# Jaroan/Contracts-MARL-AAM-Corridors

Hardware: AMD Instinct MI355X
Metric: env-steps/sec (whole node) at 4096 envs x 10 agents, navigation_graph (higher is better)
Workload: dtype f64

## Files before the change

contracts-marl-aam-corridors_amd/csrc/gmpe_kernel.h:

```cpp
#pragma once
#include <hip/hip_runtime.h>
#include <math.h>
#include <stdio.h>
#include <stdlib.h>
#include <string.h>

#include <string>
#include <utility>
#include <vector>

#include "gmpe_device.h"

namespace gmpe {

enum { MODE_STEP = 0, MODE_RESET = 1 };
enum { SC_NAV = 0, SC_NAV_WALLS = 1, SC_JULY = 2, SC_ROT = 3, SC_TWO = 4, SC_THREE = 5, SC_COUNT = 6 };
__host__ __device__ constexpr bool sc_kinematic(int sc) { return sc >= SC_JULY; }
__host__ __device__ constexpr bool sc_rotfam(int sc) { return sc >= SC_ROT; }
__host__ __device__ constexpr bool sc_phasefam(int sc) { return sc == SC_TWO || sc == SC_THREE; }

struct KParams {
    gmpe_config c;
    DevState s;
    gmpe_outputs o;
// ... 224 lines not shown
        base = k;
        const int64_t kk = k + i;
        double val;
        if (p.s.tape) val = kk < p.s.tape_len ? p.s.tape[(size_t)n * p.s.tape_len + kk] : __builtin_nan("");
        else val = philox_uniform(p.c.seed, (uint32_t)(p.c.env_id_base + n), (uint64_t)kk);
        __builtin_amdgcn_fence(__ATOMIC_ACQUIRE, "wavefront");
        buf[i] = val;
        __builtin_amdgcn_fence(__ATOMIC_RELEASE, "wavefront");
        __builtin_amdgcn_wave_barrier();
        __builtin_amdgcn_fence(__ATOMIC_ACQUIRE, "wavefront");
    }
    double v = buf[(int)(k - base)];
    if (v != v) { err |= 1; v = 0.5; }
    return v;
}

__device__ __forceinline__ bool closer_than(double dx, double dy, double thr) {
    const double d2 = dx * dx + dy * dy, t2 = thr * thr;
    if (d2 < t2 * (1.0 - 1e-12)) return true;
    if (d2 > t2 * (1.0 + 1e-12)) return false;
    return sqrt(d2) < thr;
}
__device__ __forceinline__ double draw_raw(const KParams& p, int n, int64_t k) {
    if (p.s.tape) return k < p.s.tape_len ? p.s.tape[(size_t)n * p.s.tape_len + k] : 0.5;
    return philox_uniform(p.c.seed, (uint32_t)(p.c.env_id_base + n), (uint64_t)k);
}
__device__ __forceinline__ void wave_lds_sync() {
    __builtin_amdgcn_fence(__ATOMIC_RELEASE, "wavefront");
    __builtin_amdgcn_wave_barrier();
    __builtin_amdgcn_fence(__ATOMIC_ACQUIRE, "wavefront");
}
struct DrawBuf { const double* d; int64_t base; int nd; };
__device__ __forceinline__ double buf_get(const KParams& p, const DrawBuf& w, int n, int64_t k) {
    const int64_t o = k - w.base;
    return o < w.nd ? w.d[o] : draw_raw(p, n, k);
}
__device__ __forceinline__ void place_uniform(const KParams& p, const Lds& l, const DrawBuf& win, int n, int i, bool mine, unsigned long long emask, int M, int base, double thr,
                                              bool check_static, bool is_agent, int64_t& ctr, int& err) {
    const gmpe_config& c = p.c;
    const int A = p.A, O = p.O, o0 = p.A + p.L;
    const double ws = c.world_size, size = c.entity_size, lo = -ws / 2, hi = ws / 2;
    const int lane0 = emask ? __ffsll((long long)emask) - 1 : 0;
    double* cx = l.vox; double* cy = l.voy;
    unsigned long long* cm = reinterpret_cast<unsigned long long*>(l.vnx);
    int k = 0, tries = 0;
    while (__ballot(mine && k < M)) {
        if (mine && k < M) {
            const double px = 0.8 * (lo + (hi - lo) * buf_get(p, win, n, ctr + 2 * i));
            const double py = 0.8 * (lo + (hi - lo) * buf_get(p, win, n, ctr + 2 * i + 1));
            bool bad0 = false;
            if (check_static) {
                bad0 = wall_band_hit(p, px, py, size);
                for (int o = 0; o < O; ++o) bad0 = bad0 || closer_than(l.ex[o0 + o] - px, l.ey[o0 + o] - py, 2.0 * (size + size));
            }
            for (int q = 0; q < k; ++q) bad0 = bad0 || closer_than(l.ex[base + q] - px, l.ey[base + q] - py, thr);
            cx[i] = px; cy[i] = py;
            wave_lds_sync();
            unsigned long long cl = 0ull;
            for (int j = 0; j < i; ++j) if (closer_than(cx[j] - px, cy[j] - py, thr)) cl |= 1ull << j;
            cm[i] = cl;
            wave_lds_sync();
            const unsigned long long bad = (__ballot(bad0) & emask) >> lane0;
            unsigned long long acc = 0ull;
            int kk = k, t = tries, used = 0, slot = -1;
            for (int j = 0; j < A && kk < M; ++j) {
                const bool b = ((bad >> j) & 1ull) || (cm[j] & acc) != 0ull;
                used = j + 1;
                if (b && ++t < GMPE_MAX_TRIES) continue;
                if (b) err |= 2;
                if (j == i) slot = kk;
                acc |= 1ull << j; ++kk; t = 0;
            }
            wave_lds_sync();
            if (slot >= 0) {
                l.ex[base + slot] = px; l.ey[base + slot] = py;
                if (is_agent) { l.n2[slot] = 0.0; l.n3[slot] = 0.0; }
            }
            wave_lds_sync();
            ctr += 2 * used; k = kk; tries = t;
        }
    }
}

template <int SC, bool BATCH = false>
__device__ __forceinline__ void reset_world_coop(const KParams& p, const Lds& l, int n, int i, bool mine, unsigned long long emask, int64_t& ctr, int& err) {
    const gmpe_config& c = p.c;
    const double ws = c.world_size, size = c.entity_size;
    const int A = p.A, L = p.L, O = p.O;
    const int o0 = A + L;
    int64_t wbase = -(int64_t)A - 1;
    const int64_t ctr_in = ctr;
    const DrawBuf win = {reinterpret_cast<const double*>(l.M), ctr, BATCH ? (p.E * p.E + 3) / 4 * 2 : 0};
    const int lane0 = emask ? __ffsll((long long)emask) - 1 : 0;
#define WDRAW(k) (BATCH ? buf_get(p, win, n, (k)) : win_draw(p, l.serr, wbase, A, n, i, (k), err))
    if (sc_kinematic(SC)) {
        double entx = 0, enty = 0, exx = 0, exy = 0, sa = 0, ca = 1;
        if (mine) {
            (void)WDRAW(ctr++);
            const double a = 3 * size * 2.5, b = ws * 0.15;
            const double width = a > b ? a : b;
            const double angle = -M_PI / 2 + (M_PI / 2 - (-M_PI / 2)) * WDRAW(ctr++);
            double tl = ws * 0.8;
            if (sc_phasefam(SC)) tl += -ws * 0.3 + (ws * 0.1 - (-ws * 0.3)) * WDRAW(ctr++);
            ca = cos(angle); sa = sin(angle);
            const double be = tl / 4, bx = -tl / 4;
            entx = ca * 0 + sa * be; enty = -sa * 0 + ca * be;
            exx = ca * 0 + sa * bx; exy = -sa * 0 + ca * bx;
            const double dx = exx - entx, dy = exy - enty;
            const double Lt = sqrt(dx * dx + dy * dy) + 1e-9;
            const double ex = dx / Lt, ey = dy / Lt;
            if (i == 0) {
                double* t = l.tube;
                t[T_ANGLE] = angle; t[T_ENTX] = entx; t[T_ENTY] = enty; t[T_EXX] = exx; t[T_EXY] = exy;
                t[T_EX] = ex; t[T_EY] = ey; t[T_NX] = (double)(float)(-ey); t[T_NY] = (double)(float)ex;
                t[T_L] = Lt; t[T_HALFW] = width * 0.5; t[T_WIDTH] = width;
                for (int q = 0; q < GMPE_TUBE_STRIDE; ++q) p.s.tube[(size_t)n * GMPE_TUBE_STRIDE + q] = t[q];
            }
        }
        int k = 0, tries = 0;
        double mx = 0, my = 0;
        if constexpr (BATCH) while (__ballot(mine && k < A)) {
            if (mine && k < A) {
                const double u0 = buf_get(p, win, n, ctr + 2 * i), u1 = buf_get(p, win, n, ctr + 2 * i + 1);
                constexpr bool rot = sc_rotfam(SC);
                const double jf = rot ? 0.3 : 0.2;
                const double jx = jf * (-ws + (ws - (-ws)) * u0), jy = jf * (-ws + (ws - (-ws)) * u1);
                const double dfe = rot ? (ws + k) / 3 : (ws + k) / 5;
                const double px = entx + dfe * sa + jx, py = enty + dfe * ca + jy;
                bool bad_i = wall_band_hit(p, px, py, size);
                for (int o = 0; o < O; ++o) bad_i = bad_i || closer_than(l.ex[o0 + o] - px, l.ey[o0 + o] - py, 2.0 * (size + size));
                for (int q = 0; q < k; ++q) bad_i = bad_i || closer_than(l.ex[q] - px, l.ey[q] - py, c.sep_dist);
                const unsigned long long all = emask >> lane0;
                const unsigned long long good = ~((__ballot(bad_i) & emask) >> lane0) & all;
                const int jg = good ? __ffsll((long long)good) - 1 : A;
                const int jfo = GMPE_MAX_TRIES - 1 - tries;
                int js;
                if (jfo < A && jfo < jg) { js = jfo; err |= 2; }
                else if (jg < A) js = jg;
                else { tries += A; ctr += 2 * A; continue; }
                ctr += 2 * (js + 1);
                const double th = 0.0 + (2 * M_PI - 0.0) * buf_get(p, win, n, ctr); ++ctr;
                if (i == js) { l.ex[k] = px; l.ey[k] = py; l.n2[k] = th; l.n3[k] = c.v_min; }
                wave_lds_sync();
                ++k; tries = 0;
            }
        }
        else while (__ballot(mine && k < A)) {
            if (mine && k < A) {
                const double u0 = WDRAW(ctr), u1 = WDRAW(ctr + 1);
                ctr += 2;
                constexpr bool rot = sc_rotfam(SC);
                const double jf = rot ? 0.3 : 0.2;
                const double jx = jf * (-ws + (ws - (-ws)) * u0), jy = jf * (-ws + (ws - (-ws)) * u1);
                const double dfe = rot ? (ws + k) / 3 : (ws + k) / 5;
                const double px = entx + dfe * sa + jx, py = enty + dfe * ca + jy;
                bool bad_i = wall_band_hit(p, px, py, size);
                for (int o = i; o < O; o += A) bad_i = bad_i || norm2(l.ex[o0 + o] - px, l.ey[o0 + o] - py) < 2.0 * (size + size);
                bad_i = bad_i || (i < k && norm2(mx - px, my - py) < c.sep_dist);
                const bool bad = (__ballot(bad_i) & emask) != 0ull;
                if (bad && ++tries < GMPE_MAX_TRIES) continue;
                if (bad) err |= 2;
                const double th = 0.0 + (2 * M_PI - 0.0) * WDRAW(ctr++);
                if (i == k) { mx = px; my = py; l.ex[k] = px; l.ey[k] = py; l.n2[k] = th; l.n3[k] = c.v_min; }
                ++k; tries = 0;
            }
        }
        if (mine) {
            if (c.formation_type == GMPE_FORMATION_LINE) {
                const int div = L - 1;
                const double s0 = -ws / 2, e0 = ws / 2, ddx = e0 - s0, ddy = s0 - s0;
                for (int q = i; q < L; q += A) {
                    const double f = div > 0 ? (double)q / (double)div : (double)q;
                    double lx = f * ddx + s0, ly = f * ddy + s0;
                    if (L > 1 && q == L - 1) { lx = e0; ly = s0; }
                    bool hit = wall_band_hit(p, lx, ly, size);
                    for (int o = 0; o < O; ++o) hit = hit || norm2(l.ex[o0 + o] - lx, l.ey[o0 + o] - ly) < 2.0 * (size + size);
                    if (hit) err |= 2;
                    l.ex[A + q] = lx; l.ey[A + q] = ly;
                }
            } else if (c.formation_type == GMPE_FORMATION_CIRCLE) {
                const double cy = exy + ws / 5, radius = ws / 3, angle_step = 2 * M_PI / L;
                for (int q = i; q < L; q += A) {
                    const double ang = q * angle_step;
                    l.ex[A + q] = 0.0 + radius * cos(ang); l.ey[A + q] = cy + radius * sin(ang);
                }
            } else {
                const double rel = -ws / 3;
                const double rx = ca * 0.0 + sa * rel, ry = -sa * 0.0 + ca * rel;
                for (int q = i; q < L; q += A) { l.ex[A + q] = exx + rx; l.ey[A + q] = exy + ry; }
            }
        }
    } else if constexpr (BATCH) {
        place_uniform(p, l, win, n, i, mine, emask, O, o0, 2.0 * (size + size), false, false, ctr, err);
        place_uniform(p, l, win, n, i, mine, emask, A, 0, c.sep_dist, true, true, ctr, err);
        place_uniform(p, l, win, n, i, mine, emask, L, A, c.sep_dist, true, false, ctr, err);
        if (mine) for (int o = i; o < O; o += A) {
            p.s.obstacles[((size_t)n * O + o) * 2] = l.ex[o0 + o];
            p.s.obstacles[((size_t)n * O + o) * 2 + 1] = l.ey[o0 + o];
        }
    } else {
        const double lo = -ws / 2, hi = ws / 2;
        int k = 0, tries = 0;
        while (__ballot(mine && k < O)) {
            if (mine && k < O) {
                const double px = 0.8 * (lo + (hi - lo) * WDRAW(ctr));
                const double py = 0.8 * (lo + (hi - lo) * WDRAW(ctr + 1));
                ctr += 2;
                bool bad_i = false;
                for (int q = i; q < k; q += A) bad_i = bad_i || norm2(l.ex[o0 + q] - px, l.ey[o0 + q] - py) < 2.0 * (size + size);
                const bool bad = (__ballot(bad_i) & emask) != 0ull;
                if (bad && ++tries < GMPE_MAX_TRIES) continue;
                if (bad) err |= 2;
                if (k % A == i) { l.ex[o0 + k] = px; l.ey[o0 + k] = py; }
                ++k; tries = 0;
            }
        }
        k = 0; tries = 0;
        double mx = 0, my = 0;
        while (__ballot(mine && k < A)) {
            if (mine && k < A) {
                const double px = 0.8 * (lo + (hi - lo) * WDRAW(ctr));
                const double py = 0.8 * (lo + (hi - lo) * WDRAW(ctr + 1));
                ctr += 2;
                bool bad_i = wall_band_hit(p, px, py, size);
                for (int o = i; o < O; o += A) bad_i = bad_i || norm2(l.ex[o0 + o] - px, l.ey[o0 + o] - py) < 2.0 * (size + size);
                bad_i = bad_i || (i < k && norm2(mx - px, my - py) < c.sep_dist);
                const bool bad = (__ballot(bad_i) & emask) != 0ull;
                if (bad && ++tries < GMPE_MAX_TRIES) continue;
                if (bad) err |= 2;
                if (i == k) { mx = px; my = py; l.ex[k] = px; l.ey[k] = py; l.n2[k] = 0.0; l.n3[k] = 0.0; }
                ++k; tries = 0;
            }
        }
        k = 0; tries = 0;
        while (__ballot(mine && k < L)) {
            if (mine && k < L) {
                const double px = 0.8 * (lo + (hi - lo) * WDRAW(ctr));
                const double py = 0.8 * (lo + (hi - lo) * WDRAW(ctr + 1));
                ctr += 2;
                bool bad_i = wall_band_hit(p, px, py, size);
                for (int o = i; o < O; o += A) bad_i = bad_i || norm2(l.ex[o0 + o] - px, l.ey[o0 + o] - py) < 2.0 * (size + size);
                for (int r = i; r < k; r += A) bad_i = bad_i || norm2(l.ex[A + r] - px, l.ey[A + r] - py) < c.sep_dist;
                const bool bad = (__ballot(bad_i) & emask) != 0ull;
                if (bad && ++tries < GMPE_MAX_TRIES) continue;
                if (bad) err |= 2;
                if (k % A == i) { l.ex[A + k] = px; l.ey[A + k] = py; }
                ++k; tries = 0;
            }
        }
        if (mine) for (int o = i; o < O; o += A) {
            p.s.obstacles[((size_t)n * O + o) * 2] = l.ex[o0 + o];
            p.s.obstacles[((size_t)n * O + o) * 2 + 1] = l.ey[o0 + o];
        }
    }
    if (mine) for (int q = i; q < L; q += A) {
        p.s.landmarks[((size_t)n * L + q) * 2] = l.ex[A + q];
        p.s.landmarks[((size_t)n * L + q) * 2 + 1] = l.ey[A + q];
    }
    if (BATCH && mine && p.s.tape && ctr > ctr_in && ctr > p.s.tape_len) err |= 1;
}
#undef WDRAW


template <int BLOCK, int U, int CA>
__device__ __forceinline__ void distance_trip(const KParams& p, const Lds& l, int q0, int total, int W, int dv, bool even, bool only_reset) {
    const int A = CA ? CA : p.A, E = CA ? 2 * CA : p.E, AE = A * E, EE4 = (E * E + 3) / 4 * 4;
    double ds[U]; int gs[U], rs[U], cs[U];
#pragma unroll
    for (int u = 0; u < U; ++u) {
        const int q = q0 + u * BLOCK;
        const bool live = q < total;
        const int qq = live ? q : 0;
        const int g = fdiv(qq, W, p.m_W), w = qq - g * W;
        const int a = fdiv(w, dv, p.m_Sx), b = w - a * dv;
        int r, cc;
        if (even) { const bool up = b >= a; r = up ? a : E - 1 - a; cc = up ? b + 1 : E - a + b; }
        else { int c0 = a + 1 + b; c0 = c0 >= E ? c0 - E : c0; r = a < c0 ? a : c0; cc = a < c0 ? c0 : a; }
        const double dx = l.ex[g * E + r] - l.ex[g * E + cc], dy = l.ey[g * E + r] - l.ey[g * E + cc];
// ... 201 lines not shown
            const int ab = gg * A, eb = gg * E;
            const bool kag = k < A;
            const int kk = kag ? k : 0;
            const float kx = (float)l.ex[eb + k], ky = (float)l.ey[eb + k];
            const float kvox = kag ? (float)l.vox[ab + kk] : 0.0f, kvoy = kag ? (float)l.voy[ab + kk] : 0.0f;
            const float kvnx = kag ? (float)l.vnx[ab + kk] : 0.0f, kvny = kag ? (float)l.vny[ab + kk] : 0.0f;
            const float gxk = SC == SC_TWO ? (float)l.tube[gg * GMPE_TUBE_STRIDE + T_EXX] : (kag ? (float)l.ex[eb + A + kk] : 0.0f);
            const float gyk = SC == SC_TWO ? (float)l.tube[gg * GMPE_TUBE_STRIDE + T_EXY] : (kag ? (float)l.ey[eb + A + kk] : 0.0f);
            const float typ = kag ? 0.0f : (k < A + L ? 1.0f : 2.0f);
            for (int ei = 0; ei < A; ++ei) {
                const float apx = (float)l.ex[eb + ei], apy = (float)l.ey[eb + ei];
                const float avx = (float)l.vnx[ab + ei], avy = (float)l.vny[ab + ei];
                const double cs = l.cn[ab + ei], sn = l.sn[ab + ei];
                const bool post = k <= ei;
                const float rvx = (post ? kvnx : kvox) - avx, rvy = (post ? kvny : kvoy) - avy;
                const float rpx = kx - apx, rpy = ky - apy;
                double o0, o1, o2, o3, o4, o5;
                rot2(cs, sn, (double)rvx, (double)rvy, o0, o1);
                rot2(cs, sn, (double)rpx, (double)rpy, o2, o3);
                if (kag) rot2(cs, sn, (double)(gxk - apx), (double)(gyk - apy), o4, o5); else { o4 = o2; o5 = o3; }
                float* dst = base + ((size_t)(gg * A + ei) * E + k) * 7;
                dst[0] = (float)o0; dst[1] = (float)o1; dst[2] = (float)o2; dst[3] = (float)o3;
                dst[4] = (float)o4; dst[5] = (float)o5; dst[6] = typ;
            }
        }
    }
    if (o.node_obs && !(abl & 2) && p.c.graph_feat_type == 1) {
        float* base = o.node_obs + (size_t)n0 * A * E * 7;
        for (int sidx = t0; sidx < Gv * E; sidx += nthr) {
            const int gg = fdiv(sidx, E, p.m_E), k = sidx - gg * E;
            if (!l.flags[gg * 4 + 3]) continue;
            const int ab = gg * A, eb = gg * E;
            const bool kag = k < A;
            const int kk = kag ? k : 0;
            const float kx = (float)l.ex[eb + k], ky = (float)l.ey[eb + k];
            const float kvox = kag ? (float)l.vox[ab + kk] : 0.0f, kvoy = kag ? (float)l.voy[ab + kk] : 0.0f;
            const float kvnx = kag ? (float)l.vnx[ab + kk] : 0.0f, kvny = kag ? (float)l.vny[ab + kk] : 0.0f;
            const float gx = kag ? (float)l.ex[eb + A + kk] : kx, gy = kag ? (float)l.ey[eb + A + kk] : ky;
            const float typ = kag ? 0.0f : (k < A + L ? 1.0f : 2.0f);
            for (int ei = 0; ei < A; ++ei) {
                const bool post = k <= ei;
                float* dst = base + ((size_t)(gg * A + ei) * E + k) * 7;
                dst[0] = post ? kvnx : kvox; dst[1] = post ? kvny : kvoy; dst[2] = kx; dst[3] = ky; dst[4] = gx; dst[5] = gy; dst[6] = typ;
            }
        }
    }
    if (!sc_rotfam(SC) && o.node_obs && !(abl & 2) && p.c.graph_feat_type != 1) {
        float4* base = reinterpret_cast<float4*>(o.node_obs + (size_t)n0 * A * E * GMPE_NODE_FEATS);
        const int E2 = 2 * E;
        for (int sidx = t0; sidx < Gv * E2; sidx += nthr) {
            const int gg = fdiv(sidx, E2, p.m_2E), rem = sidx - gg * E2;
            if (!l.flags[gg * 4 + 3]) continue;
            const int k = rem >> 1, half = rem & 1;
            const int ab = gg * A, eb = gg * E;
            const double kx = l.ex[eb + k], ky = l.ey[eb + k];
            const bool kag = k < A;
            const int kk = kag ? k : 0;
            const double kvox = kag ? l.vox[ab + kk] : 0.0, kvoy = kag ? l.voy[ab + kk] : 0.0;
            const double kvnx = kag ? l.vnx[ab + kk] : 0.0, kvny = kag ? l.vny[ab + kk] : 0.0;
            const double gx = kag ? l.ex[eb + A + kk] : kx, gy = kag ? l.ey[eb + A + kk] : ky;
            const float occ = kag ? 0.0f : 1.0f, typ = kag ? 0.0f : (k < A + L ? 1.0f : 2.0f);
            float4* dst = base + (size_t)gg * A * E2 + rem;
            SWEEP(ei, A) {
                const bool ok = !AP || ei < A;
                const int ec = ok ? ei : 0;
                const double px = l.ex[eb + ec], py = l.ey[eb + ec];
                float4 val;
                if (half == 0) {
                    const double evx = l.vnx[ab + ec], evy = l.vny[ab + ec];
                    const bool post = k <= ec;
                    val = make_float4((float)((post ? kvnx : kvox) - evx), (float)((post ? kvny : kvoy) - evy), (float)(kx - px), (float)(ky - py));
                } else {
                    val = make_float4((float)(gx - px), (float)(gy - py), occ, typ);
                }
                if (ok) { if (nt) nt_store4(&dst[(size_t)ec * E2], val); else dst[(size_t)ec * E2] = val; }
            }
        }
    }
}

#ifndef GMPE_BATCHED_PLACEMENT
#define GMPE_BATCHED_PLACEMENT 1
#endif
#ifndef GMPE_MIN_WAVES
#define GMPE_MIN_WAVES 1
#endif
#ifndef GMPE_MIN_WAVES_NOWALLS
#define GMPE_MIN_WAVES_NOWALLS 1
#endif

template <int BLOCK, int AP, int SC, int FL, int GC = 0>
__global__ __launch_bounds__(BLOCK, (SC == SC_NAV_WALLS ? GMPE_MIN_WAVES : (FL == 2 && BLOCK > 64 ? ((sc_rotfam(SC) || (AP > 0 && sc_kinematic(SC))) ? 3 : 4) : (AP > 0 && BLOCK > 64 ? ((sc_rotfam(SC) && !(GC > 0 && SC != SC_TWO)) ? 3 : 4) : GMPE_MIN_WAVES_NOWALLS)))) void k_env(const KParams p_arg) {
    const KParams& p = p_arg;
    constexpr bool WALLS = SC == SC_NAV_WALLS;
    extern __shared__ __attribute__((aligned(16))) char smem[];
    {
        const int __attribute__((address_space(4)))* ka = (const int __attribute__((address_space(4)))*)__builtin_amdgcn_kernarg_segment_ptr();
        int acc = 0;
#pragma unroll
        for (int q = 0; q < (int)((sizeof(KParams) + 63) / 64); ++q) acc ^= ka[q * 16];
        asm volatile("" :: "s"(acc));
    }
    const int tid = threadIdx.x;
    constexpr bool CT = AP > 0 && SC != SC_NAV_WALLS;
    const int A = CT ? AP : p.A, L = CT ? AP : p.L, O = CT ? 0 : p.O, E = CT ? 2 * AP : p.E, D = CT ? (SC == SC_JULY ? 19 : (sc_phasefam(SC) ? 15 : 13)) : p.D, G = GC > 0 ? GC : p.G, N = p.c.num_envs;
    const gmpe_config& c = p.c;
    const Lds l = carve(smem, G, A, E, D, SC == SC_NAV_WALLS ? p.c.num_walls : 0, p.nfuse);
    const int n0 = p.env_lo + blockIdx.x * G;
    const int Gv = min(G, p.env_hi - n0);
    constexpr bool july = SC == SC_JULY, rotinv = SC == SC_ROT, rotfam = sc_rotfam(SC), two = SC == SC_TWO, three = SC == SC_THREE;
    constexpr int PV = two ? 1 : (three ? 2 : 0);
    const bool step = FL ? true : p.mode == MODE_STEP;
    constexpr bool kin = sc_kinematic(SC);
    constexpr bool BATCHK = FL == 2 && AP > 0 && BLOCK > 64 && !sc_rotfam(SC) && SC != SC_NAV_WALLS && GMPE_BATCHED_PLACEMENT;
    const int EE = E * E, EE4 = (EE + 3) / 4 * 4, AD4 = (A * D + 3) / 4 * 4;
    const double INF = __builtin_huge_val();

    const int g = fdiv(tid, A, p.m_A), i = tid - g * A;
    const int n = n0 + g;
    bool ag = tid < Gv * A;
    if (ag && !step && p.mask && !p.mask[n]) ag = false;
    const size_t na = (size_t)n * A + i;
    const Lds v = env_view(l, ag ? g : 0, A, E, D);

    int prev_phase = 0, phase_reached = 0, cooldown = 0;
    double p_dist = 0, tim = 0;
    int cur_step = 0, act_idx = 0;
    int err = 0;
    int64_t ctr0 = 0;

    STAMP(0);
    const bool t_ok = tid < Gv * GMPE_TUBE_STRIDE, l_ok = tid < Gv * L, o_ok = tid < Gv * O;
    double tube0 = 0, lmx0 = 0, lmy0 = 0, obx0 = 0, oby0 = 0;
    if (t_ok) tube0 = p.s.tube[(size_t)n0 * GMPE_TUBE_STRIDE + tid];
    if (l_ok) { lmx0 = p.s.landmarks[((size_t)n0 * L + tid) * 2]; lmy0 = p.s.landmarks[((size_t)n0 * L + tid) * 2 + 1]; }
    if (o_ok) { obx0 = p.s.obstacles[((size_t)n0 * O + tid) * 2]; oby0 = p.s.obstacles[((size_t)n0 * O + tid) * 2 + 1]; }
    const int lt = BLOCK > 64 ? tid - 64 : tid;
    const bool loader = step && lt >= 0 && lt < Gv * A;
    int c9[9] = {-1, -1, -1, -1, 0, 0, 0, 0, 0}; double cd0 = 0, cd1 = 0, cds = 0;
    if (loader) {
        const size_t nl = (size_t)n0 * A + lt;
        c9[0] = p.s.times_required[nl]; c9[1] = p.s.dists_to_goal[nl]; c9[2] = p.s.dist_left[nl]; c9[3] = p.s.goal_reached[nl];
        c9[4] = p.s.n_agent_coll[nl]; c9[5] = p.s.n_obst_coll[nl]; c9[6] = p.s.spacing_viol[nl]; c9[7] = p.s.steps_in_corr[nl];
        c9[8] = p.s.conformance[nl];
        cd0 = p.s.goal_min_time[nl];
        if (SC == SC_ROT) cd1 = p.s.prev_proj[nl];
        const int lg = fdiv(lt, A, p.m_A);
        if (lt == lg * A) cds = p.s.delta_spacing[n0 + lg];
    }
    double x0 = 0, y0 = 0, a20 = 0, a30 = 0; int st0 = 0, gt0 = -1;
    if (ag) {
        prev_phase = p.s.prev_phase[na];
        cur_step = p.s.current_step[n];
        ctr0 = p.s.rng_ctr[n];
        if (step) {
            x0 = p.s.x[na]; y0 = p.s.y[na]; a20 = p.s.s2[na]; a30 = p.s.s3[na];
            st0 = p.s.status[na]; gt0 = p.s.goal_tracker[na];
            phase_reached = p.s.phase_reached[na]; cooldown = p.s.cooldown[na];
            p_dist = p.s.p_dist[na]; tim = p.s.time[na];
            if (p.act) act_idx = p.act[na];
            else {
                const float* oh = p.onehot + na * c.n_actions;
                float best = oh[0];
                for (int q = 1; q < c.n_actions; ++q) { const float x = oh[q]; if (x > best) { best = x; act_idx = q; } }
            }
        }
    }
    for (int q = tid; q < G * E; q += BLOCK) l.moff[q] = 0;
    for (int q = tid; q < A * A; q += BLOCK) {
        const int a = fdiv(q, A, p.m_A), k = q - a * A;
        if (k > a) l.ptab[a * A - a * (a + 1) / 2 + (k - a - 1)] = (a << 8) | k;
    }
    if (tid < G) {
        const int nn = n0 + tid;
        const bool active = nn < p.env_hi && (step || !p.mask || p.mask[nn]);
        l.flags[tid * 4 + 0] = (!step && active); l.flags[tid * 4 + 1] = 0; l.flags[tid * 4 + 2] = 0; l.flags[tid * 4 + 3] = active;
    }
    if (t_ok) l.tube[tid] = tube0;
    for (int q = tid + BLOCK; q < Gv * GMPE_TUBE_STRIDE; q += BLOCK) l.tube[q] = p.s.tube[(size_t)n0 * GMPE_TUBE_STRIDE + q];
    if (l_ok) { const int gg = fdiv(tid, L, p.m_L), k = tid - gg * L; l.ex[gg * E + A + k] = lmx0; l.ey[gg * E + A + k] = lmy0; }
    for (int q = tid + BLOCK; q < Gv * L; q += BLOCK) {
        const int gg = fdiv(q, L, p.m_L), k = q - gg * L;
        l.ex[gg * E + A + k] = p.s.landmarks[((size_t)n0 * L + q) * 2]; l.ey[gg * E + A + k] = p.s.landmarks[((size_t)n0 * L + q) * 2 + 1];
    }
    if (o_ok) { const int gg = fdiv(tid, O, p.m_O), k = tid - gg * O; l.ex[gg * E + A + L + k] = obx0; l.ey[gg * E + A + L + k] = oby0; }
    for (int q = tid + BLOCK; q < Gv * O; q += BLOCK) {
        const int gg = fdiv(q, O, p.m_O), k = q - gg * O;
        l.ex[gg * E + A + L + k] = p.s.obstacles[((size_t)n0 * O + q) * 2]; l.ey[gg * E + A + L + k] = p.s.obstacles[((size_t)n0 * O + q) * 2 + 1];
    }
    if (loader) {
#pragma unroll
        for (int k = 0; k < 9; ++k) l.cnt[lt * 9 + k] = c9[k];
        l.cntd[lt * 2] = cd0; l.cntd[lt * 2 + 1] = cd1;
        const int lg = fdiv(lt, A, p.m_A);
        if (lt == lg * A) l.cntd[(size_t)G * A * 2 + lg] = cds;
    }
    if (ag && step) {
// ... 134 lines not shown
                    else { vx += (sx / 1.0) * c.dt; vy += (sy / 1.0) * c.dt; }
                    if (c.max_speed > 0) {
                        const double sp = sqrt(vx * vx + vy * vy);
                        if (sp > c.max_speed) { vx = vx / sp * c.max_speed; vy = vy / sp * c.max_speed; }
                    }
                    nv2 = vx; nv3 = vy;
                    nx += vx * c.dt; ny += vy * c.dt;
                    const double ax = vx * c.dt, ay = vy * c.dt;
                    p_dist += sqrt(ax * ax + ay * ay); tim += c.dt;
                }
                v.ex[i] = nx; v.ey[i] = ny; v.s2[i] = nv2; v.s3[i] = nv3;
            }
            __syncthreads();
            STAMP(3);
            if constexpr (FUSE_OK) {
                if (FUSE) distance_force_pass<BLOCK, AP, !kin>(p, l, G, Gv, tid, false, kk == 0);
                else distance_pass<BLOCK, (CT ? AP : 0)>(p, l, Gv, tid, false);
            } else distance_pass<BLOCK, (CT ? AP : 0)>(p, l, Gv, tid, false);
            __syncthreads();
            STAMP(4);

            prevA = prev_phase;
            if (ag) {
                const double px = v.ex[i], py = v.ey[i];
                double vx, vy; vel_of<SC>(v.s2[i], v.s3[i], vx, vy);
                v.vox[i] = vx; v.voy[i] = vy;
                if (july) {
                    ph1 = phase_eval(v.tube, px, py, prev_phase, prevA);
                    if (cooldown > 0) cooldown -= 1;
                    int prevB;
                    cp = phase_eval(v.tube, px, py, prevA, prevB);
                    if (cooldown > 0) cooldown -= 1;
                    prevA = prevB;
                    goal_branch = (cp == 2 && phase_reached != 0);
                } else if (rotfam) {
                    ph1 = phase_eval_rot<PV>(v.tube, px, py, prev_phase, phase_reached);
                    if (cooldown > 0) cooldown -= 1;
                    if (cooldown > 0) cooldown -= 1;
                    cp = ph1;
                    goal_branch = (cp == 2) && (rotinv ? phase_reached >= 1 : true);
                }
                dgoal = v.Dm[(size_t)i * E + A + i];
                if (two) v.newf[i] = cp == 2 && prev_phase == 1 && phase_reached == 1 && !v.s_old[i];
                else v.newf[i] = goal_branch && dgoal < c.goal_thresh && !v.s_old[i];
            }
            if (tid < 64) {
                const unsigned long long bal = __ballot(ag && v.newf[i]);
                if (ag) {
                    if (v.newf[i]) {
                        const int rank = __popcll(bal & emask & ((1ull << tid) - 1ull));
                        if (kin) { v.n2[i] = 0.0 + (2 * M_PI - 0.0) * draw_at(c, p.s, n, ctr0 + rank, err); v.n3[i] = c.v_min; }
                        else { v.n2[i] = 0.0; v.n3[i] = 0.0; }
                        if (!two && !three) v.gt[i] = i;
                        double vx, vy; vel_of<SC>(v.n2[i], v.n3[i], vx, vy);
                        v.vnx[i] = vx; v.vny[i] = vy;
                    } else { v.n2[i] = v.s2[i]; v.n3[i] = v.s3[i]; v.vnx[i] = v.vox[i]; v.vny[i] = v.voy[i]; }
                    if (rotfam) { double sn_, cn_; sincos(v.n2[i], &sn_, &cn_); v.cn[i] = cn_; v.sn[i] = sn_; }
                    ndraw = kin ? __popcll(bal & emask) : 0;
                    if (i == 0) v.flags[1] = ndraw;
                    const bool st_now = v.s_old[i] || v.newf[i];
                    done = st_now || cur_step >= c.episode_length;
                    v.moff[i] = st_now ? 1 : 0; v.moff[A + i] = (v.gt[i] == i) ? 1 : 0;
                }
                const unsigned long long dbal = __ballot(ag && done);
                const unsigned long long mbal = __ballot(ag && (v.moff[i] | v.moff[A + i]));
                all_done = ag && ((dbal & emask) == emask);
                if (ag && i == 0) { v.flags[0] = all_done; v.flags[2] = (mbal & emask) != 0ull; }
                if (BATCHK && all_done && i == 0) reinterpret_cast<long long*>(l.cntd + (size_t)G * A * 2 + G)[g] = ctr0 + ndraw;
            }
            __syncthreads();
            STAMP(5);
        }


        int any_reset = 0, any_mask = 0;
        for (int gg = 0; gg < Gv; ++gg) { any_reset |= l.flags[gg * 4 + 0]; any_mask |= l.flags[gg * 4 + 2]; }
        const int abl = FL ? 0 : GMPE_ABL(p);

        const bool early = step && !any_reset;
        const bool spec = early && BLOCK > 64 && (FL ? true : p.spec != 0);
        if (early && !spec) stream_graph_fn<BLOCK, AP, SC, FL>(p, out, l, Gv, n0, tid, tid, BLOCK, true, any_mask);
        if constexpr (BATCHK) if (any_reset && tid >= 64) {
            const int ND = EE4 / 2;
            for (int q = tid - 64; q < Gv * ND; q += BLOCK - 64) {
                const int gg = q / ND, d = q - gg * ND;
                if (!l.flags[gg * 4 + 0]) continue;
                const int64_t c0 = reinterpret_cast<const long long*>(l.cntd + (size_t)G * A * 2 + G)[gg];
                reinterpret_cast<double*>(l.M + (size_t)gg * EE4)[d] = draw_raw(p, n0 + gg, c0 + d);
            }
        }
        if (spec) {
            if (any_mask && !(abl & 4)) {
                for (int q = tid; q < Gv * EE; q += BLOCK) {
                    const int gg = fdiv(q, EE, p.m_EE), rc = q - gg * EE;
                    if (!l.flags[gg * 4 + 2]) continue;
                    const int r = fdiv(rc, E, p.m_E), cc = rc - r * E;
                    if (l.moff[gg * E + r] | l.moff[gg * E + cc]) l.M[(size_t)gg * EE4 + rc] = 0.0f;
                }
            }
            __syncthreads();
        }
        if (step) {
            if (!spec || tid < 64) {
                const bool block_sync = !spec;
                rew = 0;
                if (ag) {
                    {
                        const int* ci = l.cnt + (size_t)(g * A + i) * 9;
                        trq = ci[0]; dtg = ci[1]; dleft = ci[2]; greached = ci[3]; nac = ci[4]; noc = ci[5]; sv = ci[6]; sic = ci[7]; conf = ci[8];
                        gmt = l.cntd[(size_t)(g * A + i) * 2]; if (rotinv) pproj = l.cntd[(size_t)(g * A + i) * 2 + 1];
                        dsp0 = l.cntd[(size_t)G * A * 2 + g];
                    }
                    const double px = v.ex[i], py = v.ey[i];
                    const double* row = v.Dm + (size_t)i * E;
                    if (rotfam) write_obs_rot<AP, SC>(p, v, i, ph1); else write_obs<AP, SC>(p, v, i, v.vox[i], v.voy[i], ph1);
                    STAMP(13);
                    int ncol_r = 0, ncol_i = 0;
                    const bool me_old = v.s_old[i] != 0, me_new = v.newf[i] != 0;
                    if (AP) {
                        double rv[AP ? AP : 1]; int so[AP ? AP : 1], nf[AP ? AP : 1];
        #pragma unroll
                        for (int a = 0; a < AP; ++a) { const int ac = a < A ? a : 0; rv[a] = row[ac]; so[a] = v.s_old[ac]; nf[a] = v.newf[ac]; }
                        __builtin_amdgcn_sched_barrier(0);
        #pragma unroll
                        for (int a = 0; a < AP; ++a) {
                            const bool close = a < A && rv[a] < c.sep_dist && a != i;
                            ncol_r += (close && !so[a] && !(nf[a] && a < i)) ? 1 : 0;
                            ncol_i += (close && !so[a] && !(nf[a] && a <= i)) ? 1 : 0;
                        }
                    } else {
                        for (int a = 0; a < A; ++a) {
                            const bool close = row[a] < c.sep_dist && a != i;
                            const int so = v.s_old[a], nf = v.newf[a];
                            ncol_r += (close && !so && !(nf && a < i)) ? 1 : 0;
                            ncol_i += (close && !so && !(nf && a <= i)) ? 1 : 0;
                        }
                    }
                    if (me_old) { ncol_r = 0; }
                    if (me_old || me_new) ncol_i = 0;
                    if (three) { for (int q = 0; q < ncol_r; ++q) rew -= c.collision_rew; }
                    else if (!two) for (int q = 0; q < ncol_r; ++q) rew -= c.collision_rew * 4;
                    nac += ncol_i;
                    STAMP(14);
                    const bool obst_hit = obstacle_collision_ego(p, v, i);
                    if (obst_hit) { if (!two && !three) rew -= c.collision_rew * 3; noc += 1; }
                    double serr = 0;
                    if (july) {
                        const double tdx = v.tube[T_EXX] - v.tube[T_ENTX], tdy = v.tube[T_EXY] - v.tube[T_ENTY];
                        const double tlen = sqrt(tdx * tdx + tdy * tdy);
                        if (cp == 2 && cp > prevA + 1) rew -= c.goal_rew * 3;
                        const double ux = tdx / tlen, uy = tdy / tlen;
                        const double qx = px - v.tube[T_ENTX], qy = py - v.tube[T_ENTY];
                        const double proj = qx * ux + qy * uy;
                        if (cp == prevA + 1 && phase_reached == cp - 1) {
                            if (cp == 1) {
                                const double edist = norm2(qx - proj * tdx, qy - proj * tdy);
                                if (0 <= proj && proj < 0.1 * tlen && edist < 0.2 * tlen) rew += c.goal_rew * 3;
                            } else if (cp == 2) rew += c.goal_rew * 3;
                        }
                        if (cp == 0) rew -= norm2(v.tube[T_ENTX] - px, v.tube[T_ENTY] - py);
                        else if (cp == 1) {
                            double hx, hy; sincos(v.s2[i], &hy, &hx);
                            int front = -1, back = -1; double fproj = 0, bproj = 0;
                            for (int k = 0; k < A; ++k) {
                                if (k == i) continue;
                                const double pj = (v.ex[k] - px) * hx + (v.ey[k] - py) * hy;
                                if (pj > 0) { if (front < 0 || pj < fproj) { front = k; fproj = pj; } }
                                else { if (back < 0 || pj > bproj) { back = k; bproj = pj; } }
                            }
                            if (front >= 0) { const double df = row[front] - c.sep_dist; serr += df < 0 ? fabs(df) : 0; }
                            if (back >= 0) { const double df = row[back] - c.sep_dist; serr += df < 0 ? fabs(df) : 0; }
                            if (serr > 0) sv += 1;
// ... 104 lines not shown
                    if (ROLL) {
                        if (p.masks) p.masks[(size_t)slot * p.st_mask + na] = done ? 0.0f : 1.0f;
                        if (p.active) p.active[(size_t)slot * p.st_mask + na] = (done && !all_done) ? 0.0f : 1.0f;
                    }
                    if (out.info) {
                        double sd = 0, st = 0, sdd = 0, stt = 0; int ssv = 0;
                        SWEEP(a, A) {
                            const bool ok = !AP || a < A;
                            const int ac = ok ? a : 0;
                            const bool nw = ac <= i;
                            const int dn = v.dtg_n[ac], d_o = v.dtg_o[ac], tn = v.trq_n[ac], to = v.trq_o[ac], svn = v.sv_n[ac], svo = v.sv_o[ac];
                            const double dd = ok ? (double)(nw ? dn : d_o) : 0.0, tt = ok ? (double)(nw ? tn : to) : 0.0;
                            sd += dd; st += tt; sdd += dd * dd; stt += tt * tt;
                            ssv += ok ? (nw ? svn : svo) : 0;
                        }
                        double dsp = dsp0;
                        if (july || rotfam) for (int a = 0; a <= i; ++a) dsp += v.serr[a];
                        const double dm = sd / A, tm = st / A;
                        const double dvn = (double)A * sdd - sd * sd, tvn = (double)A * stt - st * st;
                        const double ds = sqrt(dvn) / A, ts = sqrt(tvn) / A;
                        float* o = out.info + na * GMPE_INFO_KEYS;
                        o[0] = (float)rew; o[1] = (float)dleft; o[2] = (float)trq; o[3] = (float)nac; o[4] = (float)noc;
                        o[5] = (float)dm; o[6] = (float)ds; o[7] = (float)(dm / (ds + 0.0001)); o[8] = (float)dtg;
                        o[9] = (float)trq; o[10] = (float)tm; o[11] = (float)ts; o[12] = (float)(tm / (ts + 0.0001));
                        o[13] = (float)((double)conf / c.episode_length);
                        o[14] = (float)(dsp / (ssv != 0 ? (double)ssv : 1.0));
                        o[15] = (float)((double)sv / (sic != 0 ? sic : 1));
                        o[16] = (float)gmt;
                        o[17] = (float)phase_reached;
                    }
                    if (ROLL && !all_done && kk + 1 < K) {
                        int* ci = l.cnt + (size_t)(g * A + i) * 9;
                        ci[0] = trq; ci[1] = dtg; ci[2] = dleft; ci[3] = greached; ci[4] = nac; ci[5] = noc; ci[6] = sv; ci[7] = sic; ci[8] = conf;
                        if (rotinv) l.cntd[(size_t)(g * A + i) * 2 + 1] = pproj;
                        if (i == 0) {
                            double dsp = dsp0;
                            if (july || rotfam) for (int a = 0; a < A; ++a) dsp += v.serr[a];
                            l.cntd[(size_t)G * A * 2 + g] = dsp;
                        }
                    } else if (!all_done) {
                        if (i == 0) {
                            double dsp = dsp0;
                            if (july || rotfam) for (int a = 0; a < A; ++a) dsp += v.serr[a];
                            p.s.delta_spacing[n] = dsp;
                            p.s.rng_ctr[n] = ctr0 + v.flags[1];
                            p.s.current_step[n] = cur_step;
                        }
                        p.s.x[na] = v.ex[i]; p.s.y[na] = v.ey[i]; p.s.s2[na] = v.n2[i]; p.s.s3[na] = v.n3[i];
                        p.s.status[na] = (uint8_t)(v.s_old[i] || v.newf[i]);
                        p.s.prev_phase[na] = prev_phase; p.s.phase_reached[na] = phase_reached; p.s.cooldown[na] = cooldown;
                        p.s.goal_tracker[na] = v.gt[i]; p.s.p_dist[na] = p_dist; p.s.time[na] = tim;
                        p.s.times_required[na] = trq; p.s.dists_to_goal[na] = dtg; p.s.dist_left[na] = dleft;
                        p.s.goal_reached[na] = greached; p.s.n_agent_coll[na] = nac; p.s.n_obst_coll[na] = noc;
                        p.s.spacing_viol[na] = sv; p.s.steps_in_corr[na] = sic; p.s.conformance[na] = conf;
                        if (rotinv) p.s.prev_proj[na] = pproj;
                    }
                }
                STAMP(7);
                if (spec && !ROLL) {
                    __builtin_amdgcn_fence(__ATOMIC_RELEASE, "wavefront");
                    __builtin_amdgcn_wave_barrier();
                    __builtin_amdgcn_fence(__ATOMIC_ACQUIRE, "wavefront");
                    if (out.obs) {
                        float* dst = out.obs + (size_t)n0 * A * D;
                        const int AD = A * D;
                        for (int q = tid; q < Gv * AD; q += 64) { const int gg = fdiv(q, AD, p.m_AD); if (l.flags[gg * 4 + 3]) dst[q] = l.obs[(size_t)gg * AD4 + (q - gg * AD)]; }
                    }
                    if (out.agent_id) for (int q = tid; q < Gv * A; q += 64) { const int gg = fdiv(q, A, p.m_A); if (l.flags[gg * 4 + 3]) out.agent_id[(size_t)n0 * A + q] = q - gg * A; }
                }
            }
            else {
                STAMP_T(9, 64); STAMP_T(17, 192);
                stream_graph_fn<BLOCK, AP, SC, FL>(p, out, l, Gv, n0, tid, tid - 64, BLOCK - 64, false, any_mask);
                STAMP_T(10, 64); STAMP_T(18, 192);
            }
            __syncthreads();
        }
        {
            if (any_reset) {
                const bool mine = ag && v.flags[0];
                if (tid < 64) {
                    int64_t ctr = ctr0 + ((mine && step) ? v.flags[1] : 0);
                    STAMP(20);
                    reset_world_coop<SC, BATCHK>(p, v, n, i, mine, emask, ctr, err);
                    STAMP(21);
                    if (mine && i == 0) {
                        if (ROLL) reinterpret_cast<long long*>(l.cntd + (size_t)G * A * 2 + G)[g] = ctr;
                        p.s.rng_ctr[n] = ctr;
                        p.s.current_step[n] = 0;
                        p.s.delta_spacing[n] = 0.0;
                        v.flags[2] = 0;
                    }
                }
                __syncthreads();
                if (mine) {
                    v.s2[i] = v.n2[i]; v.s3[i] = v.n3[i];
                    double vx, vy; vel_of<SC>(v.n2[i], v.n3[i], vx, vy);
                    v.vox[i] = v.vnx[i] = vx; v.voy[i] = v.vny[i] = vy;
                    v.s_old[i] = 0; v.newf[i] = 0; v.gt[i] = -1; v.moff[i] = 0; v.moff[A + i] = 0;
                    int prevA = prev_phase, ph = 0;
                    if (july) ph = phase_eval(v.tube, v.ex[i], v.ey[i], prev_phase, prevA);
                    prev_phase = prevA;
                    if (rotfam) { ph = phase_eval_rot<PV>(v.tube, v.ex[i], v.ey[i], prev_phase, 0); double sn_, cn_; sincos(v.n2[i], &sn_, &cn_); v.cn[i] = cn_; v.sn[i] = sn_; p.s.prev_proj[na] = 0.0; }
                    const double dx = v.ex[i] - v.ex[A + i], dy = v.ey[i] - v.ey[A + i];
                    gmt = c.max_speed > 0 ? sqrt(dx * dx + dy * dy) / c.max_speed : 0.0;
                    p.s.x[na] = v.ex[i]; p.s.y[na] = v.ey[i]; p.s.s2[na] = v.n2[i]; p.s.s3[na] = v.n3[i];
                    p.s.status[na] = 0; p.s.prev_phase[na] = prev_phase; p.s.phase_reached[na] = 0; p.s.cooldown[na] = 0;
                    p.s.goal_tracker[na] = -1; p.s.p_dist[na] = 0.0; p.s.time[na] = 0.0;
                    p.s.times_required[na] = -1; p.s.dists_to_goal[na] = -1; p.s.dist_left[na] = -1;
                    p.s.goal_reached[na] = -1; p.s.n_agent_coll[na] = 0; p.s.n_obst_coll[na] = 0;
                    p.s.spacing_viol[na] = 0; p.s.steps_in_corr[na] = 0; p.s.conformance[na] = 0;
                    p.s.goal_min_time[na] = gmt;
                    ph1 = ph;
                }
                STAMP(22);
                __syncthreads();
                if constexpr (FUSE_OK) {
                    if (FUSE) distance_force_pass<BLOCK, AP, !kin>(p, l, G, Gv, tid, true, true);
                    else distance_pass<BLOCK, (CT ? AP : 0)>(p, l, Gv, tid, true);
                } else distance_pass<BLOCK, (CT ? AP : 0)>(p, l, Gv, tid, true);
                __syncthreads();
                STAMP(23);
                if (mine) { if (rotfam) write_obs_rot<AP, SC>(p, v, i, ph1); else write_obs<AP, SC>(p, v, i, v.vox[i], v.voy[i], ph1); }
                any_mask = 0;
                for (int gg = 0; gg < Gv; ++gg) any_mask |= l.flags[gg * 4 + 2];
            }
            STAMP(8);
        }
        if (ROLL && !early) {
            __builtin_amdgcn_fence(__ATOMIC_RELEASE, "workgroup");
            __syncthreads();
        }
        if (!early) stream_graph_fn<BLOCK, AP, SC, FL>(p, out, l, Gv, n0, tid, tid, BLOCK, true, any_mask);
        STAMP(11);
        if (!spec || ROLL) {
            if (out.obs) {
                float* dst = out.obs + (size_t)n0 * A * D;
                const int AD = A * D;
                for (int q = tid; q < Gv * AD; q += BLOCK) { const int gg = fdiv(q, AD, p.m_AD); if (l.flags[gg * 4 + 3]) dst[q] = l.obs[(size_t)gg * AD4 + (q - gg * AD)]; }
            }
            if (out.agent_id) for (int q = tid; q < Gv * A; q += BLOCK) { const int gg = fdiv(q, A, p.m_A); if (l.flags[gg * 4 + 3]) out.agent_id[(size_t)n0 * A + q] = q - gg * A; }
        }
        if (ROLL && kk + 1 < K) {
            if (!early) __builtin_amdgcn_fence(__ATOMIC_RELEASE, "workgroup");
            if (!spec || !early) __syncthreads();
            if (ag) {
                if (all_done) {
                    phase_reached = 0; cooldown = 0; p_dist = 0.0; tim = 0.0; cur_step = 0;
                    ctr0 = reinterpret_cast<const long long*>(l.cntd + (size_t)G * A * 2 + G)[g];
                    int* ci = l.cnt + (size_t)(g * A + i) * 9;
                    ci[0] = -1; ci[1] = -1; ci[2] = -1; ci[3] = -1; ci[4] = 0; ci[5] = 0; ci[6] = 0; ci[7] = 0; ci[8] = 0;
                    l.cntd[(size_t)(g * A + i) * 2] = gmt; l.cntd[(size_t)(g * A + i) * 2 + 1] = 0.0;
                    if (i == 0) l.cntd[(size_t)G * A * 2 + g] = 0.0;
                } else {
                    v.s2[i] = v.n2[i]; v.s3[i] = v.n3[i];
                    v.s_old[i] = (v.s_old[i] || v.newf[i]) ? 1 : 0;
                    ctr0 += ndraw;
                }
                const int na_ = c.n_actions;
                act_idx = act_next < 0 ? 0 : (act_next >= na_ ? na_ - 1 : act_next);
            }
            for (int q = tid; q < G * E; q += BLOCK) l.moff[q] = 0;
            if (tid < G) {
                const bool active = n0 + tid < p.env_hi;
                l.flags[tid * 4 + 0] = 0; l.flags[tid * 4 + 1] = 0; l.flags[tid * 4 + 2] = 0; l.flags[tid * 4 + 3] = active;
            }
            slot = slot + 1 == p.num_slots ? 0 : slot + 1;
// ... 17 lines not shown
```

Measured before the change: 209.3 million.

## Precompute navigation reset placements with wave-parallel conflict scan on helper waves

For the plain navigation scenario with batched placement, helper waves now draw 64 candidate positions per resetting env (one per lane) and resolve rejection-sampling conflicts with a ballot/readlane scan. Accepted agent and landmark positions are written to scratch LDS. The reset path then just copies those positions instead of running the serial place_uniform loops, and falls back to the old path if the window of candidates runs out. This moves the latency-bound sequential placement off the critical wave and overlaps it with the random-draw fill. In exchange it adds complexity, reuses the F2 buffer as scratch, and needs careful tolerance handling for distance comparisons near the separation threshold so results stay identical.

Result: no change. 208.7 million (-0.3%).

```diff
diff --git a/contracts-marl-aam-corridors_amd/csrc/gmpe_kernel.h b/contracts-marl-aam-corridors_amd/csrc/gmpe_kernel.h
--- a/contracts-marl-aam-corridors_amd/csrc/gmpe_kernel.h
+++ b/contracts-marl-aam-corridors_amd/csrc/gmpe_kernel.h
@@ -330,8 +330,58 @@
     }
 }
 
-template <int SC, bool BATCH = false>
-__device__ __forceinline__ void reset_world_coop(const KParams& p, const Lds& l, int n, int i, bool mine, unsigned long long emask, int64_t& ctr, int& err) {
+#ifndef GMPE_CONFLICT_C
+#define GMPE_CONFLICT_C 64
+#endif
+static_assert(GMPE_CONFLICT_C >= 2 && GMPE_CONFLICT_C <= 64 && GMPE_CONFLICT_C < GMPE_MAX_TRIES, "one lane and one mask bit per candidate; no forced accept inside the window");
+__device__ __forceinline__ double readlane_f64(double v, int lane) {
+    return __hiloint2double(__builtin_amdgcn_readlane(__double2hiint(v), lane), __builtin_amdgcn_readlane(__double2loint(v), lane));
+}
+__device__ __forceinline__ void place_by_conflicts(const KParams& p, int n, int64_t c0, int lane, int nd, double* db, double* res) {
+    const int A = p.A;
+    const double ws = p.c.world_size, lo = -ws / 2, hi = ws / 2, thr = p.c.sep_dist;
+    const double t2 = thr * thr, t_lo = t2 * (1.0 - 1e-12), t_hi = t2 * (1.0 + 1e-12);
+    double u0 = 0.5, u1 = 0.5;
+    if (2 * lane + 1 < nd) {
+        u0 = draw_raw(p, n, c0 + 2 * lane); u1 = draw_raw(p, n, c0 + 2 * lane + 1);
+        db[2 * lane] = u0; db[2 * lane + 1] = u1;
+    }
+    const double px = 0.8 * (lo + (hi - lo) * u0), py = 0.8 * (lo + (hi - lo) * u1);
+    const unsigned long long window = GMPE_CONFLICT_C >= 64 ? ~0ull : (1ull << (GMPE_CONFLICT_C & 63)) - 1ull;
+    unsigned long long blocked = 0ull;
+    int cur = 0, mine = -1;
+    for (int e = 0; e < 2 * A; ++e) {
+        if (e == A) blocked = 0ull;
+        const unsigned long long avail = cur < 64 ? (~blocked & window & (~0ull << cur)) : 0ull;
+        if (!avail) { cur = -1; break; }
+        const int j = __ffsll((long long)avail) - 1;
+        const double dx = readlane_f64(px, j) - px, dy = readlane_f64(py, j) - py;
+        const double d2 = dx * dx + dy * dy;
+        bool close = d2 < t_lo;
+        const bool edge = !close && !(d2 > t_hi);
+        if (__ballot(edge)) {
+            asm volatile("" ::: "memory");
+            close = close || (edge && sqrt(d2) < thr);
+        }
+        blocked |= __ballot(close);
+        if (lane == j) mine = e;
+        cur = j + 1;
+    }
+    if (cur >= 0 && mine >= 0) { res[mine < A ? mine : A + mine] = px; res[mine < A ? A + mine : 2 * A + mine] = py; }
+    if (lane == 0) reinterpret_cast<long long*>(res)[4 * A] = cur;
+}
+__device__ __forceinline__ bool take_placement(const KParams& p, const Lds& l, const double* res, int i, int64_t& ctr) {
+    const int A = p.A;
+    const long long used = reinterpret_cast<const long long*>(res)[4 * A];
+    if (used < 0) return false;
+    l.ex[i] = res[i]; l.ey[i] = res[A + i]; l.n2[i] = 0.0; l.n3[i] = 0.0;
+    l.ex[A + i] = res[2 * A + i]; l.ey[A + i] = res[3 * A + i];
+    ctr += 2 * used;
+    return true;
+}
+
+template <int SC, bool BATCH = false, bool CONF = false>
+__device__ __forceinline__ void reset_world_coop(const KParams& p, const Lds& l, int n, int i, bool mine, unsigned long long emask, int64_t& ctr, int& err, const double* res = nullptr) {
     const gmpe_config& c = p.c;
     const double ws = c.world_size, size = c.entity_size;
     const int A = p.A, L = p.L, O = p.O;
@@ -439,9 +489,11 @@
             }
         }
     } else if constexpr (BATCH) {
-        place_uniform(p, l, win, n, i, mine, emask, O, o0, 2.0 * (size + size), false, false, ctr, err);
-        place_uniform(p, l, win, n, i, mine, emask, A, 0, c.sep_dist, true, true, ctr, err);
-        place_uniform(p, l, win, n, i, mine, emask, L, A, c.sep_dist, true, false, ctr, err);
+        bool todo = mine;
+        if constexpr (CONF) if (res && mine) todo = !take_placement(p, l, res, i, ctr);
+        place_uniform(p, l, win, n, i, todo, emask, O, o0, 2.0 * (size + size), false, false, ctr, err);
+        place_uniform(p, l, win, n, i, todo, emask, A, 0, c.sep_dist, true, true, ctr, err);
+        place_uniform(p, l, win, n, i, todo, emask, L, A, c.sep_dist, true, false, ctr, err);
         if (mine) for (int o = i; o < O; o += A) {
             p.s.obstacles[((size_t)n * O + o) * 2] = l.ex[o0 + o];
             p.s.obstacles[((size_t)n * O + o) * 2 + 1] = l.ey[o0 + o];
@@ -809,6 +861,9 @@
 #ifndef GMPE_BATCHED_PLACEMENT
 #define GMPE_BATCHED_PLACEMENT 1
 #endif
+#ifndef GMPE_CONFLICT_PLACEMENT
+#define GMPE_CONFLICT_PLACEMENT 1
+#endif
 #ifndef GMPE_MIN_WAVES
 #define GMPE_MIN_WAVES 1
 #endif
@@ -840,6 +895,7 @@
     const bool step = FL ? true : p.mode == MODE_STEP;
     constexpr bool kin = sc_kinematic(SC);
     constexpr bool BATCHK = FL == 2 && AP > 0 && BLOCK > 64 && !sc_rotfam(SC) && SC != SC_NAV_WALLS && GMPE_BATCHED_PLACEMENT;
+    constexpr bool CONFK = BATCHK && SC == SC_NAV && AP * AP >= 4 * AP + 1 && 2 * AP * AP >= 128 && GMPE_CONFLICT_PLACEMENT;
     const int EE = E * E, EE4 = (EE + 3) / 4 * 4, AD4 = (A * D + 3) / 4 * 4;
     const double INF = __builtin_huge_val();
 
@@ -1140,12 +1196,25 @@
         if (early && !spec) stream_graph_fn<BLOCK, AP, SC, FL>(p, out, l, Gv, n0, tid, tid, BLOCK, true, any_mask);
         if constexpr (BATCHK) if (any_reset && tid >= 64) {
             const int ND = EE4 / 2;
-            for (int q = tid - 64; q < Gv * ND; q += BLOCK - 64) {
-                const int gg = q / ND, d = q - gg * ND;
+            int D0 = 0;
+            if constexpr (CONFK) if (p.nfuse > 0) {
+                D0 = 128;
+                constexpr int NS = BLOCK / 64 - 1;
+                for (int gg = ((tid >> 6) - 1 + NS - (int)(blockIdx.x % NS)) % NS; gg < Gv; gg += NS) {
+                    if (!l.flags[gg * 4 + 0]) continue;
+                    const int64_t c0 = reinterpret_cast<const long long*>(l.cntd + (size_t)G * A * 2 + G)[gg];
+                    place_by_conflicts(p, n0 + gg, c0, tid & 63, ND, reinterpret_cast<double*>(l.M + (size_t)gg * EE4), l.F2 + (size_t)gg * A * A);
+                }
+                STAMP_T(24, 64);
+            }
+            const int NR = ND - D0;
+            for (int q = BLOCK - 1 - tid; q < Gv * NR; q += BLOCK - 64) {
+                const int gg = q / NR, d = D0 + (q - gg * NR);
                 if (!l.flags[gg * 4 + 0]) continue;
                 const int64_t c0 = reinterpret_cast<const long long*>(l.cntd + (size_t)G * A * 2 + G)[gg];
                 reinterpret_cast<double*>(l.M + (size_t)gg * EE4)[d] = draw_raw(p, n0 + gg, c0 + d);
             }
+            STAMP_T(25, 64);
         }
         if (spec) {
             if (any_mask && !(abl & 4)) {
@@ -1416,7 +1485,8 @@
                 if (tid < 64) {
                     int64_t ctr = ctr0 + ((mine && step) ? v.flags[1] : 0);
                     STAMP(20);
-                    reset_world_coop<SC, BATCHK>(p, v, n, i, mine, emask, ctr, err);
+                    if constexpr (CONFK) reset_world_coop<SC, true, true>(p, v, n, i, mine, emask, ctr, err, p.nfuse > 0 ? l.F2 + (size_t)(ag ? g : 0) * A * A : nullptr);
+                    else reset_world_coop<SC, BATCHK>(p, v, n, i, mine, emask, ctr, err);
                     STAMP(21);
                     if (mine && i == 0) {
                         if (ROLL) reinterpret_cast<long long*>(l.cntd + (size_t)G * A * 2 + G)[g] = ctr;
```
